# samiazirar/mvtracker

Hardware: AMD Instinct MI355X
Metric: query-points*frames/sec, 4-view 24-frame 512x512 @1024 queries (higher is better)
Workload: dtype bf16; 1 GPU; c3: 4-view synthetic 24-frame 512x512, 1024 queries, bf16 (configs[2], the metric's config); 4-view 24-frame 512x512, 1024 queries per GPU, corr K=16 x 4 levels, iters=4, 3 windows, random-init weights (seeded recipe); queries_total=1024, parallelism=query-shard x1, frame_store=bf16 rows

## Files before the change

### mvtracker_amd/csrc/block_fused.hip

```cpp
#include "common.h"
#include <stdlib.h>

namespace {

typedef __bf16 bf16x8 __attribute__((ext_vector_type(8)));
typedef __bf16 bf16x4 __attribute__((ext_vector_type(4)));
typedef unsigned u32x4 __attribute__((ext_vector_type(4)));
typedef unsigned u32x2 __attribute__((ext_vector_type(2)));

__device__ __forceinline__ void lds_barrier() {
#ifdef MVT_FULL_BARRIERS
  __syncthreads();
#else
  __builtin_amdgcn_fence(__ATOMIC_RELEASE, "workgroup", "local");
  __builtin_amdgcn_s_barrier();
  __builtin_amdgcn_fence(__ATOMIC_ACQUIRE, "workgroup", "local");
#endif
}

constexpr int NT = 512;
constexpr int C = 256;
constexpr int LDX = C + 8;
template <int NMB> struct Cfg {
  static constexpr int BM = 32 * NMB;
  static constexpr int HC = 256;
  static constexpr int JW = HC / 32;
  static constexpr int NM1 = NMB / (8 / JW);
  static constexpr int LDH = HC + 8;
  static constexpr int LDA = 296;
  static_assert(BM * LDA <= 2 * BM * LDH, "attention tile fits the H buffers");
};
constexpr int YLD = 40;
constexpr int NBIAS_DEAL = 4 * 256 + 256;
constexpr int FS = 512;

#ifdef MVT_STAMPS
__device__ unsigned long long mvt_stamp_buf[2 * 8 * 64];
#ifndef MVT_STAMP_SEL
#define MVT_STAMP_SEL true
#endif
#ifndef MVT_STAMP_WG1
#define MVT_STAMP_WG1 100
#endif
#define STAMP(i)                                                                                                  \
  do {                                                                                                            \
    __builtin_amdgcn_sched_barrier(0);                                                                            \
    unsigned long long t_;                                                                                        \
    asm volatile("s_memtime %0\n\ts_waitcnt lgkmcnt(0)" : "=s"(t_)::"memory");                                    \
    __builtin_amdgcn_sched_barrier(0);                                                                            \
    if (lane == 0 && MVT_STAMP_SEL && (bx == 0 || bx == MVT_STAMP_WG1) && by == 0 && bz == 0)  \
      mvt_stamp_buf[((bx ? 1 : 0) * 8 + wave) * 64 + (i)] = t_;                                                   \
  } while (0)
#else
#define STAMP(i) \
  do {           \
  } while (0)
#endif

#if defined(MVT_STAMPS) && defined(MVT_ASTAMPS)
#define ASTAMP(i)                                       \
  do {                                                  \
    const int wave = threadIdx.x >> 6;                  \
    const int bx = blockIdx.x, by = blockIdx.y, bz = blockIdx.z; \
    STAMP(i);                                           \
  } while (0)
#else
#define ASTAMP(i) \
  do {            \
  } while (0)
#endif

struct BlockArgs {
  float* x;
  int ldx;
  const float* att;
  int ldatt, Ko;
  const unsigned short* wo;
  const float* bo;
  int ldwo;
  const unsigned short* w1;
  const float* b1;
  const unsigned short* w2;
  const float* b2;
  int ldw1, ldw2, H;
  mvt_block_next next[MVT_BLOCK_MAX_NEXT];
  int n_next;
  int deal, deal_img[MVT_BLOCK_MAX_NEXT], deal_rep[2];
  int att_bf16;
  long long M;
  float* ws;
  const unsigned short* aq;
  const unsigned short* ak;
  const unsigned short* av;
  int ldaq, ldakv, S, nkeys, bmv;
  const float* parts;
  int nsplit;
  const float* tokx;
  const unsigned short* win;
  const float* bin;
  const float* virt;
  int ldtok;
  long long Mp;
  const float* t_coords;
  const float* t_fcorr;
  const float* t_ffeats;
  const float* t_maskvis;
  const float* t_pos;
  const float* t_time;
  int t_E, t_Fc, t_Cf, t_D;
  const float* c_ws;
  const float* c_b2;
  float* c_x;
  int c_ldx, c_nch;
  mvt_block_next c_kv;
  mvt_block_next c_next;
};

typedef float f32x2 __attribute__((ext_vector_type(2)));
__device__ __forceinline__ f32x2 gelu_tanh_pk(f32x2 x) {
  const f32x2 c0 = {-2.3022082f, -2.3022082f}, c1 = {-0.10294324f, -0.10294324f}, one = {1.0f, 1.0f};
  const f32x2 a = (x * x * c1 + c0) * x;
  f32x2 e;
  e[0] = __builtin_amdgcn_exp2f(a[0]);
  e[1] = __builtin_amdgcn_exp2f(a[1]);
  const f32x2 d = e + one;
  f32x2 rc;
  rc[0] = __builtin_amdgcn_rcpf(d[0]);
  rc[1] = __builtin_amdgcn_rcpf(d[1]);
  return x * rc;
}

__device__ __forceinline__ bf16x8 ldg_frag(const unsigned short* p) {
  return __builtin_bit_cast(bf16x8, *reinterpret_cast<const u32x4*>(p));
}
__device__ __forceinline__ bf16x8 lds_frag(const unsigned short* p) {
  return __builtin_bit_cast(bf16x8, *reinterpret_cast<const u32x4*>(p));
}

template <int KS, int NMB>
__device__ __forceinline__ void gemm_wt(f32x16 (&acc)[NMB], const unsigned short* wrow, const unsigned short* arow, int lda,
                                        int mb0) {
  constexpr int PF = (KS % 8 == 0) ? 8 : 4;
  bf16x8 wq[PF];
#pragma unroll
  for (int i = 0; i < PF; ++i) wq[i] = ldg_frag(wrow + (i < KS ? i : 0) * FS);
#pragma unroll 1
  for (int g = 0; g < KS / PF; ++g) {
#pragma unroll
    for (int j = 0; j < PF; ++j) {
      const int ks = g * PF + j;
      const bf16x8 wa = wq[j];
      wq[j] = ldg_frag(wrow + (ks + PF < KS ? ks + PF : KS - 1) * FS);
#pragma unroll
      for (int i = 0; i < NMB; ++i) {
        const bf16x8 xb = lds_frag(arow + (mb0 + i) * 32 * lda + ks * 16);
        acc[i] = __builtin_amdgcn_mfma_f32_32x32x16_bf16(wa, xb, acc[i], 0, 0, 0);
      }
    }
  }
#pragma unroll
  for (int j = 0; j < KS % PF; ++j) {
    const int ks = (KS / PF) * PF + j;
#pragma unroll
    for (int i = 0; i < NMB; ++i) {
      const bf16x8 xb = lds_frag(arow + (mb0 + i) * 32 * lda + ks * 16);
      acc[i] = __builtin_amdgcn_mfma_f32_32x32x16_bf16(wq[j], xb, acc[i], 0, 0, 0);
    }
  }
}

constexpr int PFQ = 16;
template <int KS, int NMB>
__device__ __forceinline__ void gemm_wq(f32x16 (&acc)[NMB], bf16x8 (&wq)[PFQ], const unsigned short* wrow, const unsigned short* nxt,
                                        const unsigned short* arow, int lda, int mb0) {
  static_assert(KS == PFQ, "every GEMM segment is exactly one queue length");
  constexpr int GK = NMB >= 2 ? 2 : 4;
  bf16x8 xa[GK][NMB], xn[GK][NMB];
// ... 5 lines not shown
  for (int g = 0; g < KS / GK; ++g) {
    if (g + 1 < KS / GK) {
#pragma unroll
      for (int j = 0; j < GK; ++j)
#pragma unroll
        for (int i = 0; i < NMB; ++i) xn[j][i] = lds_frag(arow + (mb0 + i) * 32 * lda + ((g + 1) * GK + j) * 16);
    }
    __builtin_amdgcn_sched_barrier(0);
#pragma unroll
    for (int j = 0; j < GK; ++j) {
      const int ks = g * GK + j;
      const bf16x8 wa = wq[ks];
#ifndef MVT_ABL_NOLOAD
      wq[ks] = ldg_frag(nxt + ks * FS);
#endif
#pragma unroll
      for (int i = 0; i < NMB; ++i) {
#ifdef MVT_ABL_NOLDS
        const bf16x8 xb = wa;
#else
        const bf16x8 xb = xa[j][i];
#endif
#ifdef MVT_ABL_NOMFMA
        acc[i][0] += (float)xb[0] + (float)wa[1];
#else
        acc[i] = __builtin_amdgcn_mfma_f32_32x32x16_bf16(wa, xb, acc[i], 0, 0, 0);
#endif
      }
    }
    __builtin_amdgcn_sched_barrier(0);
    if (g + 1 < KS / GK) {
#pragma unroll
      for (int j = 0; j < GK; ++j)
#pragma unroll
        for (int i = 0; i < NMB; ++i) xa[j][i] = xn[j][i];
    }
  }
}
template <int NMB, bool REFILL>
__device__ __forceinline__ void gemm_wq18(f32x16 (&acc)[NMB], bf16x8 (&wq)[PFQ], const bf16x8 (&wx)[2], const unsigned short* nxt,
                                          const unsigned short* arow, int lda) {
  constexpr int KS = 18, GK = 2;
  bf16x8 xa[GK][NMB], xn[GK][NMB];
#pragma unroll
  for (int j = 0; j < GK; ++j)
#pragma unroll
    for (int i = 0; i < NMB; ++i) xa[j][i] = lds_frag(arow + i * 32 * lda + j * 16);
#pragma unroll
  for (int g = 0; g < KS / GK; ++g) {
    if (g + 1 < KS / GK) {
#pragma unroll
      for (int j = 0; j < GK; ++j)
#pragma unroll
        for (int i = 0; i < NMB; ++i) xn[j][i] = lds_frag(arow + i * 32 * lda + ((g + 1) * GK + j) * 16);
    }
    __builtin_amdgcn_sched_barrier(0);
#pragma unroll
    for (int j = 0; j < GK; ++j) {
      const int ks = g * GK + j;
      const bf16x8 wa = ks < PFQ ? wq[ks < PFQ ? ks : 0] : wx[ks >= PFQ ? ks - PFQ : 0];
      if (REFILL && ks < PFQ) wq[ks] = ldg_frag(nxt + ks * FS);
#pragma unroll
      for (int i = 0; i < NMB; ++i) acc[i] = __builtin_amdgcn_mfma_f32_32x32x16_bf16(wa, xa[j][i], acc[i], 0, 0, 0);
    }
    __builtin_amdgcn_sched_barrier(0);
    if (g + 1 < KS / GK) {
#pragma unroll
      for (int j = 0; j < GK; ++j)
#pragma unroll
        for (int i = 0; i < NMB; ++i) xa[j][i] = xn[j][i];
    }
  }
}
__device__ __forceinline__ void fill_wq(bf16x8 (&wq)[PFQ], const unsigned short* wrow) {
#pragma unroll
  for (int j = 0; j < PFQ; ++j) wq[j] = ldg_frag(wrow + j * FS);
}

constexpr int LDVA = 40, DHA = 48, VTA = DHA * LDVA;
constexpr int LDKV = 584;
template <int NMBQ, int NKB> struct AttnFrags {
  u32x4 q[NMBQ][3];
  u32x4 k[NKB][3];
  u32x2 v[NKB][6];
};
template <int NMBQ, int NKB, class QR, class KR>
__device__ __forceinline__ void attn_load(AttnFrags<NMBQ, NKB>& f, const unsigned short* __restrict__ q, int ldq, QR qrow, int nq,
                                          const unsigned short* __restrict__ k, const unsigned short* __restrict__ v, int ldkv, KR krow,
                                          int nk, int hd, int lane) {
  const int r = lane & 31, h = lane >> 5;
#pragma unroll
  for (int mb = 0; mb < NMBQ; ++mb) {
    const int qi = mb * 32 + r;
    const long long qo = qrow(qi < nq ? qi : nq - 1) * (long long)ldq + hd * DHA;
#pragma unroll
    for (int ks = 0; ks < 3; ++ks) f.q[mb][ks] = *reinterpret_cast<const u32x4*>(q + qo + ks * 16 + 8 * h);
  }
#pragma unroll
  for (int kb = 0; kb < NKB; ++kb) {
    const int key = kb * 32 + r;
    const long long ko = krow(key < nk ? key : nk - 1) * (long long)ldkv + hd * DHA;
#pragma unroll
    for (int ks = 0; ks < 3; ++ks) f.k[kb][ks] = *reinterpret_cast<const u32x4*>(k + ko + ks * 16 + 8 * h);
#pragma unroll
    for (int i = 0; i < 6; ++i) f.v[kb][i] = *reinterpret_cast<const u32x2*>(v + ko + 24 * h + 4 * i);
  }
}
__device__ __forceinline__ f32x4 bf4_to_f32(unsigned lo, unsigned hi) {
  return (f32x4){__uint_as_float(lo << 16), __uint_as_float(lo & 0xFFFF0000u), __uint_as_float(hi << 16), __uint_as_float(hi & 0xFFFF0000u)};
}
__device__ __forceinline__ float pair_max(float v) {
  const auto r = __builtin_amdgcn_permlane32_swap(__float_as_int(v), __float_as_int(v), false, false);
  return fmaxf(__int_as_float(r[0]), __int_as_float(r[1]));
}
__device__ __forceinline__ float pair_sum(float v) {
  const auto r = __builtin_amdgcn_permlane32_swap(__float_as_int(v), __float_as_int(v), false, false);
  return __int_as_float(r[0]) + __int_as_float(r[1]);
}

template <int NMBQ, int NKB>
__device__ __forceinline__ void attn_compute(const AttnFrags<NMBQ, NKB>& f, int nq, int nk, int hd, unsigned short* vt,
                                             const unsigned short* zrow, unsigned short* As, int lda, int arow0, int lane, int bd = 0,
                                             int vstride = 0) {
  const int r = lane & 31, h = lane >> 5;
  const float scale = 1.0f / sqrtf((float)DHA);
  auto stage_vt = [&](int kb, unsigned short* img) {
    const int key = kb * 32 + r;
#pragma unroll
    for (int i = 0; i < 6; ++i) {
      u32x2 w = f.v[kb][i];
      if (key >= nk) w = (u32x2){0u, 0u};
#pragma unroll
      for (int e = 0; e < 4; ++e) img[(24 * h + 4 * i + e) * LDVA + r] = (unsigned short)((e & 1) ? (w[e >> 1] >> 16) : (w[e >> 1] & 0xFFFFu));
    }
  };
  if (vstride > 0) {
    __builtin_amdgcn_fence(__ATOMIC_SEQ_CST, "wavefront");
#pragma unroll
    for (int kb = 0; kb < NKB; ++kb) stage_vt(kb, vt + kb * vstride);
    __builtin_amdgcn_fence(__ATOMIC_SEQ_CST, "wavefront");
  }
  __builtin_amdgcn_sched_barrier(0);
  ASTAMP(49);
  bf16x8 qf[NMBQ][3];
#pragma unroll
  for (int mb = 0; mb < NMBQ; ++mb) {
#pragma unroll
    for (int ks = 0; ks < 3; ++ks) {
      f32x4 a = bf4_to_f32(f.q[mb][ks][0], f.q[mb][ks][1]), b = bf4_to_f32(f.q[mb][ks][2], f.q[mb][ks][3]);
#pragma unroll
      for (int e = 0; e < 4; ++e) {
        a[e] *= scale;
        b[e] *= scale;
      }
      const bf16x4 x = __builtin_convertvector(a, bf16x4), y = __builtin_convertvector(b, bf16x4);
#pragma unroll
      for (int e = 0; e < 4; ++e) {
        qf[mb][ks][e] = x[e];
        qf[mb][ks][4 + e] = y[e];
      }
    }
  }
  const unsigned bdm = bd > 0 ? (65536u / (unsigned)bd + 1u) : 0u;
#pragma unroll
  for (int mb = 0; mb < NMBQ; ++mb) {
    const int qi = mb * 32 + r;
    const unsigned qt = ((unsigned)qi * bdm) >> 16;
    f32x16 sc[NKB];
    float mx = -INFINITY;
#pragma unroll
    for (int kb = 0; kb < NKB; ++kb) {
#pragma unroll
      for (int e = 0; e < 16; ++e) sc[kb][e] = 0.f;
#pragma unroll
      for (int ks = 0; ks < 3; ++ks) sc[kb] = __builtin_amdgcn_mfma_f32_32x32x16_bf16(__builtin_bit_cast(bf16x8, f.k[kb][ks]), qf[mb][ks], sc[kb], 0, 0, 0);
    }
#pragma unroll
    for (int kb = 0; kb < NKB; ++kb) {
      const bool half = nk <= kb * 32 + 16;
#pragma unroll
      for (int e = 0; e < 16; ++e) {
        const unsigned kk = (unsigned)(kb * 32 + (e & 3) + 8 * (e >> 2)) + 4u * (unsigned)h;
        const bool ok = (kk < (unsigned)nk) & (((kk * bdm) >> 16) == qt);
        sc[kb][e] = ok ? sc[kb][e] : -INFINITY;
      }
#pragma unroll
      for (int e = 0; e < 8; ++e) mx = fmaxf(mx, sc[kb][e]);
      if (!half) {
#pragma unroll
        for (int e = 8; e < 16; ++e) mx = fmaxf(mx, sc[kb][e]);
      }
    }
    mx = pair_max(mx);
    if (mx == -INFINITY) mx = 0.f;
    float ps = 0.f;
#pragma unroll
    for (int kb = 0; kb < NKB; ++kb) {
      const bool half = nk <= kb * 32 + 16;
#pragma unroll
      for (int e = 0; e < 8; ++e) {
        sc[kb][e] = __expf(sc[kb][e] - mx);
        ps += sc[kb][e];
      }
      if (!half) {
#pragma unroll
        for (int e = 8; e < 16; ++e) {
          sc[kb][e] = __expf(sc[kb][e] - mx);
          ps += sc[kb][e];
        }
      }
    }
    __builtin_amdgcn_sched_barrier(0);
    ASTAMP(50 + 2 * mb);
    f32x16 oacc[2];
#pragma unroll
    for (int db = 0; db < 2; ++db)
#pragma unroll
      for (int e = 0; e < 16; ++e) oacc[db][e] = 0.f;
#pragma unroll
    for (int kb = 0; kb < NKB; ++kb) {
      const bool half = nk <= kb * 32 + 16;
      const unsigned short* vimg = vt + kb * vstride;
      if (vstride == 0 && (mb == 0 || NKB > 1)) {
        __builtin_amdgcn_fence(__ATOMIC_SEQ_CST, "wavefront");
        stage_vt(kb, vt);
        __builtin_amdgcn_fence(__ATOMIC_SEQ_CST, "wavefront");
      }
#pragma unroll
      for (int sk = 0; sk < 2; ++sk) {
        if (sk == 1 && half) break;
        f32x4 lo4, hi4;
#pragma unroll
        for (int e = 0; e < 4; ++e) {
          lo4[e] = sc[kb][8 * sk + e];
          hi4[e] = sc[kb][8 * sk + 4 + e];
        }
        const bf16x4 bl = __builtin_convertvector(lo4, bf16x4), bh = __builtin_convertvector(hi4, bf16x4);
        bf16x8 pb;
#pragma unroll
        for (int e = 0; e < 4; ++e) {
          pb[e] = bl[e];
          pb[4 + e] = bh[e];
        }
#pragma unroll
        for (int db = 0; db < 2; ++db) {
          const unsigned short* vr = (db * 32 + r < DHA) ? &vimg[(db * 32 + r) * LDVA + 16 * sk + 4 * h] : zrow + 16 * sk + 4 * h;
          const u32x2 a0 = *reinterpret_cast<const u32x2*>(vr), a1 = *reinterpret_cast<const u32x2*>(vr + 8);
          const bf16x8 va = __builtin_bit_cast(bf16x8, (u32x4){a0[0], a0[1], a1[0], a1[1]});
          oacc[db] = __builtin_amdgcn_mfma_f32_32x32x16_bf16(va, pb, oacc[db], 0, 0, 0);
        }
      }
    }
    __builtin_amdgcn_sched_barrier(0);
    ASTAMP(51 + 2 * mb);
    const float lt = pair_sum(ps);
    const float inv = 1.0f / lt;
    if (qi >= nq) continue;
#pragma unroll
    for (int db = 0; db < 2; ++db) {
#pragma unroll
      for (int gq = 0; gq < 4; ++gq) {
        const int d = db * 32 + 8 * gq + 4 * h;
        if (d < DHA) {
          f32x4 t;
#pragma unroll
          for (int e = 0; e < 4; ++e) t[e] = oacc[db][4 * gq + e] * inv;
          *reinterpret_cast<u32x2*>(&As[(arow0 + qi) * lda + hd * DHA + d]) = __builtin_bit_cast(u32x2, __builtin_convertvector(t, bf16x4));
        }
      }
    }
  }
}

template <int NMB>
__device__ __forceinline__ void ln_to_lds(const f32x16 (&v)[NMB], unsigned short* Xs, float* st, int wave, int lane, float eps,
                                          const float* lnw, const float* lnb, float (&ms)[NMB][2], bool have, bool sync = true) {
  constexpr int BM = 32 * NMB;
  const int r = lane & 31, h = lane >> 5;
  f32x4 gw[4], gb[4];
  if (lnw) {
#pragma unroll
    for (int g = 0; g < 4; ++g) {
      gw[g] = *reinterpret_cast<const f32x4*>(lnw + wave * 32 + 8 * g + 4 * h);
      gb[g] = *reinterpret_cast<const f32x4*>(lnb + wave * 32 + 8 * g + 4 * h);
    }
  }
  if (!have) {
#pragma unroll
    for (int mb = 0; mb < NMB; ++mb) {
      float s1 = 0.f, s2 = 0.f;
#pragma unroll
      for (int e = 0; e < 16; ++e) {
        s1 += v[mb][e];
        s2 = fmaf(v[mb][e], v[mb][e], s2);
      }
      s1 += __shfl_xor(s1, 32, 64);
      s2 += __shfl_xor(s2, 32, 64);
      if (h == 0) {
        st[(wave * BM + mb * 32 + r) * 2] = s1;
        st[(wave * BM + mb * 32 + r) * 2 + 1] = s2;
      }
    }
    lds_barrier();
#pragma unroll
    for (int mb = 0; mb < NMB; ++mb) {
      float s1 = 0.f, s2 = 0.f;
#pragma unroll
      for (int w = 0; w < 8; ++w) {
// ... 368 lines not shown
      const bool virt = m >= p.Mp;
      const long long tk = virt ? (m - p.Mp) / p.S : 0;
#pragma unroll
      for (int e = 0; e < 16; ++e) {
        const int c = wave * 32 + (e & 3) + 8 * (e >> 2) + 4 * h;
        v[mb][e] = virt ? p.virt[tk * C + c] : v[mb][e] + p.bin[c];
      }
    }
  } else if (MODE != 2 && ATT == 3) {
    unsigned short* As = &Hs[0][0];
    static_assert(ATT != 3 || NMB == 1, "partials tiles are 32 tokens");
    if (wave < 6) {
      const int mb = bx;
      const long long nchunk = (long long)p.S * 6;
      const long long cid = (long long)bz * 6 + wave;
      constexpr int MAXS = MVT_ATTN_NSPLIT;
      float ms[MAXS], ls[MAXS];
      f32x4 os[MAXS][2][4];
#pragma unroll
      for (int w = 0; w < MAXS; ++w) {
        const long long rec = (w < p.nsplit ? w : 0) * nchunk + cid;
        const f32x4 q0 = *reinterpret_cast<const f32x4*>(p.parts + mvt_part_off(rec, 0, lane));
        ms[w] = q0[mb];
        ls[w] = q0[2 + mb];
#pragma unroll
        for (int db = 0; db < 2; ++db)
#pragma unroll
          for (int g = 0; g < 4; ++g)
            os[w][db][g] = *reinterpret_cast<const f32x4*>(p.parts + mvt_part_off(rec, 1 + (mb * 2 + db) * 4 + g, lane));
      }
      __builtin_amdgcn_sched_barrier(0);
      float mm = ms[0], ll = ls[0];
      f32x16 oa[2];
#pragma unroll
      for (int db = 0; db < 2; ++db)
#pragma unroll
        for (int g = 0; g < 4; ++g)
#pragma unroll
          for (int e = 0; e < 4; ++e) oa[db][4 * g + e] = os[0][db][g][e];
#pragma unroll
      for (int w = 1; w < MAXS; ++w) {
        if (w >= p.nsplit) break;
        const float mw = ms[w];
        const float mn = fmaxf(mm, mw);
        const float ca = (mm == -INFINITY) ? 0.f : __expf(mm - mn);
        const float cb = (mw == -INFINITY) ? 0.f : __expf(mw - mn);
        ll = fmaf(ll, ca, ls[w] * cb);
#pragma unroll
        for (int db = 0; db < 2; ++db)
#pragma unroll
          for (int g = 0; g < 4; ++g)
#pragma unroll
            for (int e = 0; e < 4; ++e) oa[db][4 * g + e] = fmaf(oa[db][4 * g + e], ca, os[w][db][g][e] * cb);
        mm = mn;
      }
      const float inv = 1.0f / (ll + __shfl_xor(ll, 32, 64));
#pragma unroll
      for (int db = 0; db < 2; ++db)
#pragma unroll
        for (int g = 0; g < 4; ++g) {
          const int d = db * 32 + 8 * g + 4 * h;
          if (d < DHA) {
            f32x4 t4;
#pragma unroll
            for (int e = 0; e < 4; ++e) t4[e] = oa[db][4 * g + e] * inv;
            *reinterpret_cast<u32x2*>(&As[r * LDA + wave * DHA + d]) = __builtin_bit_cast(u32x2, __builtin_convertvector(t4, bf16x4));
          }
        }
    }
    pre_gemm();
    lds_barrier();
    gemm_wq18<NMB, HAS_MLP>(v, wq, wx, fc1_first, &As[r * LDA + 8 * h], LDA);
#pragma unroll
    for (int mb = 0; mb < NMB; ++mb)
#pragma unroll
      for (int e = 0; e < 16; ++e) v[mb][e] += p.bo[wave * 32 + (e & 3) + 8 * (e >> 2) + 4 * h];
  } else if (MODE != 2 && ATT != 0) {
    unsigned short* As = &Hs[0][0];
    unsigned short* zrow = reinterpret_cast<unsigned short*>(st);
    if (t < 48) zrow[t] = 0;
    constexpr int XW = (BM * LDX) / VTA;
    constexpr int VPW = NMB == 2 ? 2 : 1;
    constexpr int XWV = XW / VPW;
    unsigned short* vt = wave < XWV ? &Xs[wave * VPW * VTA] : &Hs[0][0] + ((BM * LDA + 7) & ~7) + (wave - XWV) * VPW * VTA;
    constexpr int vstride = VPW == 2 ? VTA : 0;
    static_assert(XWV + ((2 * BM * LDH - BM * LDA - 8) / VTA) / VPW >= 6, "the V^T images of six waves fit beside the attention tile");
    lds_barrier();
    STAMP(1);
    if (ATT == 1) {
      const long long left = p.M - m0;
      const int nrow = left < bmv ? (int)left : bmv;
      if (wave < 6 && nrow > 0) {
        auto row = [&](int j) { return m0 + j; };
        AttnFrags<NMB, 2> fr;
        attn_load<NMB, 2>(fr, p.aq, p.ldaq, row, nrow, p.ak, p.av, p.ldakv, row, nrow, wave, lane);
        attn_compute<NMB, 2>(fr, nrow, nrow, wave, vt, zrow, As, LDA, 0, lane, p.S, vstride);
      }
    } else {
      const bool on = wave < 6 && grow(0) >= 0;
      const long long left = ntok - (long long)bx * BM;
      const int nq = left < BM ? (int)left : BM;
      auto qrow = [&](int i) { return ((long long)bx * BM + i) * p.S + (long long)bz; };
      AttnFrags<NMB, 2> fr;
      if (CTX) {
        const unsigned short* KV = &Hs[0][0];
        auto krow = [&](int j) { return (long long)j; };
        if (on) attn_load<NMB, 2>(fr, p.aq, p.ldaq, qrow, nq, KV, KV + 288, LDKV, krow, p.nkeys, wave, lane);
        lds_barrier();
      } else {
        auto krow = [&](int j) { return (long long)j * p.S + (long long)bz; };
        if (on) attn_load<NMB, 2>(fr, p.aq, p.ldaq, qrow, nq, p.ak, p.av, p.ldakv, krow, p.nkeys, wave, lane);
      }
      if (on) attn_compute<NMB, 2>(fr, nq, p.nkeys, wave, vt, zrow, As, LDA, 0, lane, 0, vstride);
    }
    pre_gemm();
    STAMP(2);
    lds_barrier();
    STAMP(3);
    gemm_wq18<NMB, HAS_MLP>(v, wq, wx, fc1_first, &As[r * LDA + 8 * h], LDA);
#pragma unroll
    for (int mb = 0; mb < NMB; ++mb)
#pragma unroll
      for (int e = 0; e < 16; ++e) v[mb][e] += p.bo[wave * 32 + (e & 3) + 8 * (e >> 2) + 4 * h];
  } else if (MODE != 2 && p.att) {
    unsigned short* As = &Hs[0][0];
    const int q4 = p.Ko / 4;
    for (int f = t; f < BM * q4; f += NT) {
      const int row = f / q4, c = (f - row * q4) * 4;
      const long long m = grow(row);
      u32x2 w = (u32x2){0u, 0u};
      if (m >= 0) {
        if (p.att_bf16) {
          w = *reinterpret_cast<const u32x2*>(reinterpret_cast<const unsigned short*>(p.att) + m * (long long)p.ldatt + c);
        } else {
          const f32x4 a = *reinterpret_cast<const f32x4*>(p.att + m * (long long)p.ldatt + c);
          w = __builtin_bit_cast(u32x2, __builtin_convertvector(a, bf16x4));
        }
      }
      *reinterpret_cast<u32x2*>(&As[row * LDA + c]) = w;
    }
    pre_gemm();
    STAMP(2);
    lds_barrier();
    STAMP(3);
    gemm_wq18<NMB, HAS_MLP>(v, wq, wx, fc1_first, &As[r * LDA + 8 * h], LDA);
#pragma unroll
    for (int mb = 0; mb < NMB; ++mb)
#pragma unroll
      for (int e = 0; e < 16; ++e) v[mb][e] += p.bo[wave * 32 + (e & 3) + 8 * (e >> 2) + 4 * h];
  } else {
    load_x();
  }
  STAMP(4);
  if (MODE == 2 && p.ws) {
    constexpr int MAXCH = 4;
    const int nch = p.H / Cfg<NMB>::HC;
    f32x4 part[NMB][4][MAXCH + 1];
#pragma unroll
    for (int mb = 0; mb < NMB; ++mb) {
      const long long m = grow(mb * 32 + r);
#pragma unroll
      for (int g = 0; g < 4; ++g)
#pragma unroll
        for (int sidx = 0; sidx <= MAXCH; ++sidx)
          part[mb][g][sidx] = (m >= 0 && sidx <= nch) ? *reinterpret_cast<const f32x4*>(p.ws + ws_off(sidx, g)) : (f32x4){0.f, 0.f, 0.f, 0.f};
    }
    __builtin_amdgcn_sched_barrier(0);
#pragma unroll
    for (int mb = 0; mb < NMB; ++mb)
#pragma unroll
      for (int g = 0; g < 4; ++g) {
        f32x4 xv = part[mb][g][0];
#pragma unroll
        for (int sidx = 1; sidx <= MAXCH; ++sidx)
          if (sidx <= nch) {
#pragma unroll
            for (int e = 0; e < 4; ++e) xv[e] += part[mb][g][sidx][e];
          }
#pragma unroll
        for (int e = 0; e < 4; ++e) v[mb][4 * g + e] += xv[e] + p.b2[wave * 32 + 8 * g + 4 * h + e];
      }
  } else if (ATT != 4) {
#pragma unroll
    for (int mb = 0; mb < NMB; ++mb)
#pragma unroll
      for (int g = 0; g < 4; ++g)
#pragma unroll
        for (int e = 0; e < 4; ++e) v[mb][4 * g + e] += xr[mb][g][e];
  }

  auto store_x = [&]() {
#pragma unroll
    for (int mb = 0; mb < NMB; ++mb) {
      const long long m = grow(mb * 32 + r);
      if (m >= 0) {
#pragma unroll
        for (int g = 0; g < 4; ++g) {
          f32x4 o;
// ... 206 lines not shown
      for (int mb = 0; mb < NMB; ++mb)
#pragma unroll
        for (int e = 0; e < 16; ++e) acc[mb][e] = 0.f;
      gemm_wq<C / 16, NMB>(acc, wq, nrow_of(nb), nb + nbstep < nblocks ? nrow_of(nb + nbstep) : (chain ? chain : nrow_of(nb)), &Xs[r * LDX + 8 * h], LDX, 0);
      STAMP(34 + 8 * q + (nb - nb0) / nbstep);
      if (nx.y_bf16 && nb * 32 + 31 < nx.N && (nx.ldy & 7) == 0 && ((uintptr_t)nx.y & 15) == 0) {
        unsigned short* tile = &Hs[0][0] + wave * (NMB * 32 * YLD);
        __builtin_amdgcn_fence(__ATOMIC_SEQ_CST, "wavefront");
#pragma unroll
        for (int mb = 0; mb < NMB; ++mb)
#pragma unroll
          for (int g = 0; g < 4; ++g) {
            f32x4 o;
#pragma unroll
            for (int e = 0; e < 4; ++e) o[e] = acc[mb][4 * g + e] + b1s[nb * 32 + 8 * g + 4 * h + e];
            *reinterpret_cast<u32x2*>(&tile[(mb * 32 + r) * YLD + 8 * g + 4 * h]) = __builtin_bit_cast(u32x2, __builtin_convertvector(o, bf16x4));
          }
        __builtin_amdgcn_fence(__ATOMIC_SEQ_CST, "wavefront");
        unsigned short* yb = reinterpret_cast<unsigned short*>(nx.y) + nb * 32;
#pragma unroll
        for (int k = 0; k < NMB * 2; ++k) {
          const int pc = lane + 64 * k, row = pc >> 2, c = pc & 3;
          const long long m = grow(row);
          if (m >= nx.row_lo && m < nx.row_hi)
            *reinterpret_cast<u32x4*>(yb + m * (long long)nx.ldy + c * 8) = *reinterpret_cast<const u32x4*>(&tile[row * YLD + c * 8]);
        }
        continue;
      }
#pragma unroll
      for (int mb = 0; mb < NMB; ++mb) {
        const long long m = grow(mb * 32 + r);
        if (m < nx.row_lo || m >= nx.row_hi) continue;
#pragma unroll
        for (int g = 0; g < 4; ++g) {
          const int n = nb * 32 + 8 * g + 4 * h;
          if (n + 3 < nx.N) {
            f32x4 o;
#pragma unroll
            for (int e = 0; e < 4; ++e) o[e] = acc[mb][4 * g + e] + b1s[n + e];
            store_act4(nx.y, m * (long long)nx.ldy + n, o, nx.y_bf16);
          } else {
#pragma unroll
            for (int e = 0; e < 4; ++e)
              if (n + e < nx.N) store_act(nx.y, m * (long long)nx.ldy + n + e, acc[mb][4 * g + e] + b1s[n + e], nx.y_bf16);
          }
        }
      }
    }
    STAMP(39 + 8 * q);
  }
  STAMP(63);
}

__global__ void pack_frag_kernel(const unsigned short* __restrict__ w, int ld, int N, int K, unsigned short* __restrict__ out) {
  const long long total = (long long)((N + 31) / 32) * (K / 16) * 64;
  for (long long i = blockIdx.x * (long long)blockDim.x + threadIdx.x; i < total; i += (long long)gridDim.x * blockDim.x) {
    const int lane = (int)(i & 63);
    const long long f = i >> 6;
    const int ks = (int)(f % (K / 16));
    const int nb = (int)(f / (K / 16));
    const int n = nb * 32 + (lane & 31), k = ks * 16 + 8 * (lane >> 5);
    u32x4 v = (u32x4){0u, 0u, 0u, 0u};
    if (n < N) v = *reinterpret_cast<const u32x4*>(w + (long long)n * ld + k);
    *reinterpret_cast<u32x4*>(out + i * 8) = v;
  }
}

}

#ifdef MVT_STAMPS
extern "C" int mvt_debug_read_stamps(unsigned long long* host) {
  return hipMemcpyFromSymbol(host, HIP_SYMBOL(mvt_stamp_buf), sizeof(unsigned long long) * 2 * 8 * 64) == hipSuccess ? MVT_OK : MVT_ERR_HIP_BASE;
}
extern "C" int mvt_debug_clear_stamps() {
  static unsigned long long z[2 * 8 * 64];
  return hipMemcpyToSymbol(HIP_SYMBOL(mvt_stamp_buf), z, sizeof(z)) == hipSuccess ? MVT_OK : MVT_ERR_HIP_BASE;
}
#endif

static inline int proj_seq_switch() {
  const char* e = getenv("MVT_PROJ_SEQ");
  return e && atoi(e) != 0;
}
static void plan_deal(BlockArgs& a) {
  a.deal = 0;
  if (proj_seq_switch() || a.n_next == 0) return;
  int nimg = 0, total = 0;
  for (int q = 0; q < a.n_next; ++q) {
    const mvt_block_next& nx = a.next[q];
    if (!nx.y_bf16 || (nx.N & 31) || (nx.ldy & 7) || ((uintptr_t)nx.y & 15)) return;
    int im = -1;
    for (int qq = 0; qq < q && im < 0; ++qq)
      if (a.next[qq].lnw == nx.lnw && a.next[qq].lnb == nx.lnb && a.next[qq].eps == nx.eps) im = a.deal_img[qq];
    if (im < 0) {
      if (nimg == 2) return;
      im = nimg++;
      a.deal_rep[im] = q;
    }
    a.deal_img[q] = im;
    total += nx.N;
  }
  if (total <= NBIAS_DEAL) a.deal = 1;
}

extern "C" int mvt_pack_frag_bf16(const unsigned short* w, int ld, int N, int K, unsigned short* out, void* stream) {
  MVT_REQUIRE(w && out && N > 0 && K > 0 && K % 16 == 0 && ld % 8 == 0 && ld >= K);
  MVT_REQUIRE(((uintptr_t)w % 16 == 0) && ((uintptr_t)out % 16 == 0));
  const long long total = (long long)((N + 31) / 32) * (K / 16) * 64;
  hipLaunchKernelGGL(pack_frag_kernel, dim3((unsigned)mvt_cdiv(total, 256)), dim3(256), 0, mvt_stream(stream), w, ld, N, K, out);
  return mvt_launch_status();
}

extern "C" int mvt_block_fused_bf16(float* x, int ldx, const void* att, int att_bf16, int ldatt, int Ko, const unsigned short* wo, int ldwo,
                                    const float* bo, const unsigned short* w1, int ldw1, const float* b1, const unsigned short* w2,
                                    int ldw2, const float* b2, int H, const mvt_block_next* next, int n_next, long long M, int Cc,
                                    float* workspace, void* stream) {
  MVT_REQUIRE(x && w1 && b1 && w2 && b2 && M > 0 && Cc == C && H > 0 && H % 256 == 0 && H <= 4 * C);
  MVT_REQUIRE(ldx % 4 == 0 && ldx >= C);
  MVT_REQUIRE(!att || (wo && bo && Ko == 288 && ldatt % 4 == 0 && ldatt >= Ko));
  MVT_REQUIRE(n_next >= 0 && n_next <= MVT_BLOCK_MAX_NEXT && (n_next == 0 || next));
  MVT_REQUIRE(((uintptr_t)x % 16 == 0) && ((uintptr_t)att % 16 == 0) && ((uintptr_t)wo % 16 == 0) && ((uintptr_t)w1 % 16 == 0) &&
              ((uintptr_t)w2 % 16 == 0));
  BlockArgs a{};
  a.x = x; a.ldx = ldx; a.att = (const float*)att; a.att_bf16 = att_bf16 ? 1 : 0; a.ldatt = ldatt; a.Ko = Ko; a.wo = wo; a.bo = bo; a.ldwo = ldwo;
  a.w1 = w1; a.b1 = b1; a.w2 = w2; a.b2 = b2; a.ldw1 = ldw1; a.ldw2 = ldw2; a.H = H; a.M = M; a.n_next = n_next;
  for (int q = 0; q < n_next; ++q) {
    const mvt_block_next& nx = next[q];
    MVT_REQUIRE(nx.w && nx.b && nx.y && nx.N > 0 && nx.N <= 4 * C && nx.ldy % 4 == 0 && nx.ldy >= nx.N);
    MVT_REQUIRE(nx.y_bf16 == 0 || nx.y_bf16 == 1);
    MVT_REQUIRE((nx.lnw == nullptr) == (nx.lnb == nullptr) && ((uintptr_t)nx.lnw % 16 == 0) && ((uintptr_t)nx.lnb % 16 == 0) && ((uintptr_t)nx.w % 16 == 0) && ((uintptr_t)nx.y % 16 == 0));
    MVT_REQUIRE(nx.row_lo >= 0 && (nx.row_hi == 0 || nx.row_hi > nx.row_lo));
    a.next[q] = nx;
    if (nx.row_hi == 0) a.next[q].row_hi = M;
  }
  plan_deal(a);
  static const char* force = getenv("MVT_BLOCK_NMB");
  const int nmb = force ? atoi(force) : (M >= 4096 ? 2 : 1);
  static const bool no_split = getenv("MVT_BLOCK_NOSPLIT") != nullptr;
  a.ws = workspace;
  if (nmb == 2) {
    hipLaunchKernelGGL((block_fused_bf16<2, 0, 0>), dim3((unsigned)mvt_cdiv(M, 64)), dim3(NT), 0, mvt_stream(stream), a);
  } else if (workspace && !no_split && M <= 2048 && M % 32 == 0) {
    MVT_REQUIRE((uintptr_t)workspace % 16 == 0);
    const unsigned tiles = (unsigned)mvt_cdiv(M, 32);
    hipLaunchKernelGGL((block_fused_bf16<1, 1, 0>), dim3(tiles, (unsigned)(H / 256)), dim3(NT), 0, mvt_stream(stream), a);
    int maxblk = 1;
    for (int q = 0; q < n_next; ++q) maxblk = (next[q].N + 31) / 32 > maxblk ? (next[q].N + 31) / 32 : maxblk;
    const unsigned slices = n_next ? (unsigned)mvt_cdiv(maxblk, 8) : 1u;
    hipLaunchKernelGGL((block_fused_bf16<1, 2, 0>), dim3(tiles, slices), dim3(NT), 0, mvt_stream(stream), a);
  } else {
    hipLaunchKernelGGL((block_fused_bf16<1, 0, 0>), dim3((unsigned)mvt_cdiv(M, 32)), dim3(NT), 0, mvt_stream(stream), a);
  }
  return mvt_launch_status();
}

extern "C" int mvt_attn_block_fused_bf16(float* x, int ldx, const mvt_block_attn* attn, const unsigned short* wo, const float* bo,
                                         const unsigned short* w1, const float* b1, const unsigned short* w2, const float* b2, int H,
                                         const mvt_block_next* next, int n_next, long long M, int Cc, float* workspace, void* stream) {
  MVT_REQUIRE(x && attn && wo && bo && w1 && b1 && w2 && b2 && M > 0 && Cc == C && H > 0 && H % 256 == 0 && H <= 4 * C);
  MVT_REQUIRE(ldx % 4 == 0 && ldx >= C && n_next >= 0 && n_next <= MVT_BLOCK_MAX_NEXT && (n_next == 0 || next));
  MVT_REQUIRE(attn->heads == 6 && attn->dim_head == DHA && attn->S >= 1 && M % attn->S == 0);
  MVT_REQUIRE(attn->kind == MVT_ATTN_PARTIALS || (attn->kind == MVT_ATTN_FRAME_CTX && attn->q && attn->ldq % 8 == 0 && attn->ldq >= 288) ||
              (attn->q && attn->k && attn->v && attn->ldq % 8 == 0 && attn->ldkv % 8 == 0 && attn->ldq >= 288 && attn->ldkv >= 288));
  MVT_REQUIRE(((uintptr_t)x % 16 == 0) && ((uintptr_t)wo % 16 == 0) && ((uintptr_t)w1 % 16 == 0) && ((uintptr_t)w2 % 16 == 0));
  MVT_REQUIRE(((uintptr_t)attn->q % 16 == 0) && ((uintptr_t)attn->k % 16 == 0) && ((uintptr_t)attn->v % 16 == 0));
  BlockArgs a{};
  a.x = x; a.ldx = ldx; a.att = nullptr; a.Ko = 288; a.wo = wo; a.bo = bo; a.ldwo = 288;
  a.w1 = w1; a.b1 = b1; a.w2 = w2; a.b2 = b2; a.ldw1 = C; a.ldw2 = H; a.H = H; a.M = M; a.n_next = n_next; a.ws = workspace;
  a.aq = attn->q; a.ak = attn->k; a.av = attn->v; a.ldaq = attn->ldq; a.ldakv = attn->ldkv; a.S = attn->S; a.nkeys = attn->n_keys;
  for (int q = 0; q < n_next; ++q) {
    const mvt_block_next& nx = next[q];
    MVT_REQUIRE(nx.w && nx.b && nx.y && nx.N > 0 && nx.N <= 4 * C && nx.ldy % 4 == 0 && nx.ldy >= nx.N);
    MVT_REQUIRE((nx.y_bf16 == 0 || nx.y_bf16 == 1) && (nx.lnw == nullptr) == (nx.lnb == nullptr) && ((uintptr_t)nx.lnw % 16 == 0) && ((uintptr_t)nx.lnb % 16 == 0));
    MVT_REQUIRE(((uintptr_t)nx.w % 16 == 0) && ((uintptr_t)nx.y % 16 == 0) && nx.row_lo >= 0 && (nx.row_hi == 0 || nx.row_hi > nx.row_lo));
    a.next[q] = nx;
    if (nx.row_hi == 0) a.next[q].row_hi = M;
  }
  plan_deal(a);
  const int S = attn->S;
  if (attn->kind == MVT_ATTN_TIME) {
    MVT_REQUIRE(S <= 32 && !workspace);
    static const bool small_tiles = !(getenv("MVT_TIME_NMB1") && atoi(getenv("MVT_TIME_NMB1")) == 0);
    if (small_tiles && mvt_cdiv(M, (32 / S) * S) <= 256) {
      a.bmv = (32 / S) * S;
      hipLaunchKernelGGL((block_fused_bf16<1, 0, 1>), dim3((unsigned)mvt_cdiv(M, a.bmv)), dim3(NT), 0, mvt_stream(stream), a);
      return mvt_launch_status();
    }
    a.bmv = (64 / S) * S;
    hipLaunchKernelGGL((block_fused_bf16<2, 0, 1>), dim3((unsigned)mvt_cdiv(M, a.bmv)), dim3(NT), 0, mvt_stream(stream), a);
  } else if (attn->kind == MVT_ATTN_PARTIALS) {
    MVT_REQUIRE(attn->partials && attn->n_splits >= 1 && attn->n_splits <= MVT_ATTN_NSPLIT && attn->n_keys == 64 && M == 64LL * S);
    MVT_REQUIRE(workspace && (uintptr_t)workspace % 16 == 0 && M <= 2048 && (uintptr_t)attn->partials % 16 == 0);
    a.parts = attn->partials; a.nsplit = attn->n_splits;
    const unsigned tiles = (unsigned)mvt_cdiv(M, 32);
    a.S = S;
    hipLaunchKernelGGL((block_fused_bf16<1, 1, 3>), dim3(2, (unsigned)(H / 256), (unsigned)S), dim3(NT), 0, mvt_stream(stream), a);
    int maxblk = 1;
    for (int q = 0; q < n_next; ++q) maxblk = (next[q].N + 31) / 32 > maxblk ? (next[q].N + 31) / 32 : maxblk;
    const unsigned slices = n_next ? (unsigned)mvt_cdiv(maxblk, 8) : 1u;
    (void)tiles;
    if (!attn->defer_pass2)
      hipLaunchKernelGGL((block_fused_bf16<1, 2, 5>), dim3(2, slices, (unsigned)S), dim3(NT), 0, mvt_stream(stream), a);
  } else if (attn->kind == MVT_ATTN_FRAME) {
    MVT_REQUIRE(attn->n_keys >= 1 && attn->n_keys <= 64);
    const long long ntok = M / S;
    static const bool small_tiles = !(getenv("MVT_FRAME_NMB1") && atoi(getenv("MVT_FRAME_NMB1")) == 0);
    if (small_tiles && mvt_frame_small_tiles(ntok, S)) {
      MVT_REQUIRE(!workspace);
      hipLaunchKernelGGL((block_fused_bf16<1, 0, 2>), dim3((unsigned)mvt_cdiv(ntok, 32), 1, (unsigned)S), dim3(NT), 0, mvt_stream(stream), a);
    } else if (ntok * S >= 4096) {
      MVT_REQUIRE(!workspace);
      hipLaunchKernelGGL((block_fused_bf16<2, 0, 2>), dim3((unsigned)mvt_cdiv(ntok, 64), 1, (unsigned)S), dim3(NT), 0, mvt_stream(stream), a);
    } else {
      MVT_REQUIRE(workspace && (uintptr_t)workspace % 16 == 0 && M <= 2048 && ntok % 32 == 0);
      hipLaunchKernelGGL((block_fused_bf16<1, 1, 2>), dim3((unsigned)(ntok / 32), (unsigned)(H / 256), (unsigned)S), dim3(NT), 0,
                         mvt_stream(stream), a);
      int maxblk = 1;
      for (int q = 0; q < n_next; ++q) maxblk = (next[q].N + 31) / 32 > maxblk ? (next[q].N + 31) / 32 : maxblk;
      const unsigned slices = n_next ? (unsigned)mvt_cdiv(maxblk, 8) : 1u;
      if (!attn->defer_pass2)
        hipLaunchKernelGGL((block_fused_bf16<1, 2, 5>), dim3((unsigned)(ntok / 32), slices, (unsigned)S), dim3(NT), 0, mvt_stream(stream), a);
    }
  } else if (attn->kind == MVT_ATTN_FRAME_CTX) {
    const mvt_block_ctx* cx = attn->ctx;
    const long long ntok = M / S;
    MVT_REQUIRE(cx && attn->n_keys == 64 && ntok * S >= 4096 && !workspace && !attn->defer_pass2);
    MVT_REQUIRE(cx->ws && cx->b2 && cx->x && cx->chunks >= 1 && cx->chunks <= 4 && cx->ldx % 4 == 0 && cx->ldx >= C);
    MVT_REQUIRE(((uintptr_t)cx->ws % 16 == 0) && ((uintptr_t)cx->b2 % 16 == 0) && ((uintptr_t)cx->x % 16 == 0));
    MVT_REQUIRE(cx->kv.w && cx->kv.b && cx->kv.N == 2 * 288 && (cx->kv.lnw == nullptr) == (cx->kv.lnb == nullptr));
    MVT_REQUIRE(((uintptr_t)cx->kv.w % 16 == 0) && ((uintptr_t)cx->kv.lnw % 16 == 0) && ((uintptr_t)cx->kv.lnb % 16 == 0));
    const unsigned tiles = (unsigned)mvt_cdiv(ntok, 64);
    if (cx->next.w) {
      const mvt_block_next& nx = cx->next;
      MVT_REQUIRE(nx.b && nx.y && nx.N > 0 && nx.N <= 4 * C && nx.ldy % 4 == 0 && nx.ldy >= nx.N && (nx.y_bf16 == 0 || nx.y_bf16 == 1));
      MVT_REQUIRE((nx.lnw == nullptr) == (nx.lnb == nullptr) && ((uintptr_t)nx.lnw % 16 == 0) && ((uintptr_t)nx.lnb % 16 == 0));
      MVT_REQUIRE(((uintptr_t)nx.w % 16 == 0) && ((uintptr_t)nx.y % 16 == 0) && (nx.N + 31) / 32 <= 8 * (int)tiles);
    }
    a.c_ws = cx->ws; a.c_b2 = cx->b2; a.c_x = cx->x; a.c_ldx = cx->ldx; a.c_nch = cx->chunks; a.c_kv = cx->kv; a.c_next = cx->next;
    hipLaunchKernelGGL((block_fused_bf16<2, 0, 6>), dim3(tiles, 1, (unsigned)S), dim3(NT), 0, mvt_stream(stream), a);
  } else {
    return MVT_ERR_ARG;
  }
  return mvt_launch_status();
}

extern "C" int mvt_input_proj_bf16(const float* tokens, int ldtok, int token_dim, long long Mp, const unsigned short* win, const float* bin,
                                   const float* virtual_tokens, int S, float* x, int ldx, const mvt_block_next* next, int n_next, long long M,
                                   int Cc, void* stream) {
  MVT_REQUIRE(tokens && win && bin && virtual_tokens && x && next && n_next >= 1 && n_next <= MVT_BLOCK_MAX_NEXT && Cc == C);
  MVT_REQUIRE(M > 0 && Mp >= 0 && Mp <= M && S >= 1 && (M - Mp) % S == 0 && token_dim >= 1 && token_dim <= 37 * 16 && ldtok >= token_dim);
  MVT_REQUIRE(ldtok % 4 == 0 && ldx % 4 == 0 && ldx >= C && ((uintptr_t)tokens % 16 == 0) && ((uintptr_t)win % 16 == 0) && ((uintptr_t)x % 16 == 0));
  BlockArgs a{};
  a.x = x; a.ldx = ldx; a.M = M; a.n_next = n_next; a.H = 4 * C; a.ws = nullptr; a.S = S;
  a.tokx = tokens; a.ldtok = ldtok; a.win = win; a.bin = bin; a.virt = virtual_tokens; a.Mp = Mp;
  for (int q = 0; q < n_next; ++q) {
    const mvt_block_next& nx = next[q];
    MVT_REQUIRE(nx.w && nx.b && nx.y && nx.N > 0 && nx.N <= 4 * C && nx.ldy % 4 == 0 && nx.ldy >= nx.N);
    MVT_REQUIRE((nx.lnw == nullptr) == (nx.lnb == nullptr) && ((uintptr_t)nx.lnw % 16 == 0) && ((uintptr_t)nx.lnb % 16 == 0) && ((uintptr_t)nx.w % 16 == 0) && ((uintptr_t)nx.y % 16 == 0));
    MVT_REQUIRE(nx.row_lo >= 0 && (nx.row_hi == 0 || nx.row_hi > nx.row_lo) && (nx.y_bf16 == 0 || nx.y_bf16 == 1));
    a.next[q] = nx;
    if (nx.row_hi == 0) a.next[q].row_hi = M;
  }
  plan_deal(a);
  hipLaunchKernelGGL((block_fused_bf16<2, 3, 4>), dim3((unsigned)mvt_cdiv(M, 64)), dim3(NT), 0, mvt_stream(stream), a);
  return mvt_launch_status();
}

extern "C" int mvt_token_input_proj_bf16(const float* coords, const float* fcorr, int Fc, const float* ffeats, int Cf, const float* mask_vis,
                                         const float* pos, const float* time_embed, int n_tracks, int S, int E,
                                         const unsigned short* win, const float* bin, const float* virtual_tokens, float* x, int ldx,
                                         const mvt_block_next* next, int n_next, long long M, int Cc, void* stream) {
  MVT_REQUIRE(coords && fcorr && ffeats && mask_vis && pos && time_embed && win && bin && virtual_tokens && x && next);
  MVT_REQUIRE(n_next >= 1 && n_next <= MVT_BLOCK_MAX_NEXT && Cc == C && n_tracks > 0 && S >= 1 && E > 0 && E % 2 == 0 && Fc > 0 && Cf > 0);
  const int D = 3 * E + 3 + Fc + Cf + 2;
  const long long Mp = (long long)n_tracks * S;
  MVT_REQUIRE(D <= 37 * 16 && M >= Mp && (M - Mp) % S == 0 && ldx % 4 == 0 && ldx >= C);
  MVT_REQUIRE(((uintptr_t)win % 16 == 0) && ((uintptr_t)x % 16 == 0));
  BlockArgs a{};
  a.x = x; a.ldx = ldx; a.M = M; a.n_next = n_next; a.H = 4 * C; a.ws = nullptr; a.S = S;
  a.tokx = nullptr; a.win = win; a.bin = bin; a.virt = virtual_tokens; a.Mp = Mp;
  a.t_coords = coords; a.t_fcorr = fcorr; a.t_ffeats = ffeats; a.t_maskvis = mask_vis; a.t_pos = pos; a.t_time = time_embed;
  a.t_E = E; a.t_Fc = Fc; a.t_Cf = Cf; a.t_D = D;
  for (int q = 0; q < n_next; ++q) {
    const mvt_block_next& nx = next[q];
    MVT_REQUIRE(nx.w && nx.b && nx.y && nx.N > 0 && nx.N <= 4 * C && nx.ldy % 4 == 0 && nx.ldy >= nx.N);
    MVT_REQUIRE((nx.lnw == nullptr) == (nx.lnb == nullptr) && ((uintptr_t)nx.lnw % 16 == 0) && ((uintptr_t)nx.lnb % 16 == 0) && ((uintptr_t)nx.w % 16 == 0) && ((uintptr_t)nx.y % 16 == 0));
    MVT_REQUIRE(nx.row_lo >= 0 && (nx.row_hi == 0 || nx.row_hi > nx.row_lo) && (nx.y_bf16 == 0 || nx.y_bf16 == 1));
    a.next[q] = nx;
    if (nx.row_hi == 0) a.next[q].row_hi = M;
  }
  plan_deal(a);
  hipLaunchKernelGGL((block_fused_bf16<2, 3, 4>), dim3((unsigned)mvt_cdiv(M, 64)), dim3(NT), 0, mvt_stream(stream), a);
  return mvt_launch_status();
// ... 26 lines not shown
```

Before: 1.072 million query-points*frames/s.

## Split two attention heads across idle waves in 64-row fused block tiles

In the NMB=2 fused-block attention stage, only six of eight waves previously did head work. By default (attn_six off), waves 4-7 now split heads 4 and 5 by 32-query halves. Each cut wave stages its half of V^T and signals the partner through an LDS flag, and runs pre_gemm before its attention instead of after. V fragments are loaded as 16-byte vectors, and an env switch can force the 64-row tile path. This adds spin-wait flags and extra register and sync complexity to balance wave load.

```diff
diff --git a/mvtracker_amd/csrc/block_fused.hip b/mvtracker_amd/csrc/block_fused.hip
--- a/mvtracker_amd/csrc/block_fused.hip
+++ b/mvtracker_amd/csrc/block_fused.hip
@@ -62,7 +62,7 @@
   do {                                                  \
     const int wave = threadIdx.x >> 6;                  \
     const int bx = blockIdx.x, by = blockIdx.y, bz = blockIdx.z; \
-    STAMP(i);                                           \
+    STAMP((i) + 7);                                     \
   } while (0)
 #else
 #define ASTAMP(i) \
@@ -93,6 +93,7 @@
   const unsigned short* ak;
   const unsigned short* av;
   int ldaq, ldakv, S, nkeys, bmv;
+  int attn_six;
   const float* parts;
   int nsplit;
   const float* tokx;
@@ -264,16 +265,16 @@
 template <int NMBQ, int NKB> struct AttnFrags {
   u32x4 q[NMBQ][3];
   u32x4 k[NKB][3];
-  u32x2 v[NKB][6];
+  u32x4 v[NKB][3];
 };
 template <int NMBQ, int NKB, class QR, class KR>
 __device__ __forceinline__ void attn_load(AttnFrags<NMBQ, NKB>& f, const unsigned short* __restrict__ q, int ldq, QR qrow, int nq,
                                           const unsigned short* __restrict__ k, const unsigned short* __restrict__ v, int ldkv, KR krow,
-                                          int nk, int hd, int lane) {
+                                          int nk, int hd, int lane, int q0 = 0, int vkb = -1) {
   const int r = lane & 31, h = lane >> 5;
 #pragma unroll
   for (int mb = 0; mb < NMBQ; ++mb) {
-    const int qi = mb * 32 + r;
+    const int qi = q0 + mb * 32 + r;
     const long long qo = qrow(qi < nq ? qi : nq - 1) * (long long)ldq + hd * DHA;
 #pragma unroll
     for (int ks = 0; ks < 3; ++ks) f.q[mb][ks] = *reinterpret_cast<const u32x4*>(q + qo + ks * 16 + 8 * h);
@@ -284,8 +285,27 @@
     const long long ko = krow(key < nk ? key : nk - 1) * (long long)ldkv + hd * DHA;
 #pragma unroll
     for (int ks = 0; ks < 3; ++ks) f.k[kb][ks] = *reinterpret_cast<const u32x4*>(k + ko + ks * 16 + 8 * h);
-#pragma unroll
-    for (int i = 0; i < 6; ++i) f.v[kb][i] = *reinterpret_cast<const u32x2*>(v + ko + 24 * h + 4 * i);
+    if (vkb < 0) {
+#pragma unroll
+      for (int i = 0; i < 3; ++i) f.v[kb][i] = *reinterpret_cast<const u32x4*>(v + ko + 24 * h + 8 * i);
+    }
+  }
+  if (vkb >= 0) {
+    const int key = vkb * 32 + r;
+    const long long vo = krow(key < nk ? key : nk - 1) * (long long)ldkv + hd * DHA;
+#pragma unroll
+    for (int i = 0; i < 3; ++i) f.v[0][i] = *reinterpret_cast<const u32x4*>(v + vo + 24 * h + 8 * i);
+  }
+}
+__device__ __forceinline__ void attn_stage_vt(const u32x4 (&v)[3], int kb, int nk, unsigned short* img, int lane) {
+  const int r = lane & 31, h = lane >> 5;
+  const int key = kb * 32 + r;
+#pragma unroll
+  for (int i = 0; i < 6; ++i) {
+    u32x2 w = (u32x2){v[i >> 1][2 * (i & 1)], v[i >> 1][2 * (i & 1) + 1]};
+    if (key >= nk) w = (u32x2){0u, 0u};
+#pragma unroll
+    for (int e = 0; e < 4; ++e) img[(24 * h + 4 * i + e) * LDVA + r] = (unsigned short)((e & 1) ? (w[e >> 1] >> 16) : (w[e >> 1] & 0xFFFFu));
   }
 }
 __device__ __forceinline__ f32x4 bf4_to_f32(unsigned lo, unsigned hi) {
@@ -300,28 +320,22 @@
   return __int_as_float(r[0]) + __int_as_float(r[1]);
 }
 
+__device__ __forceinline__ void lds_flag_set(int* flag) {
+  __builtin_amdgcn_fence(__ATOMIC_RELEASE, "workgroup", "local");
+  __hip_atomic_store(flag, 1, __ATOMIC_RELAXED, __HIP_MEMORY_SCOPE_WORKGROUP);
+}
+__device__ __forceinline__ void lds_flag_wait(int* flag) {
+#pragma clang loop unroll(disable)
+  for (int i = 0; i < (1 << 20) && __hip_atomic_load(flag, __ATOMIC_RELAXED, __HIP_MEMORY_SCOPE_WORKGROUP) == 0; ++i) __builtin_amdgcn_s_sleep(1);
+  __builtin_amdgcn_fence(__ATOMIC_ACQUIRE, "workgroup", "local");
+}
+
 template <int NMBQ, int NKB>
 __device__ __forceinline__ void attn_compute(const AttnFrags<NMBQ, NKB>& f, int nq, int nk, int hd, unsigned short* vt,
                                              const unsigned short* zrow, unsigned short* As, int lda, int arow0, int lane, int bd = 0,
-                                             int vstride = 0) {
+                                             int vstride = 0, int q0 = 0, int* vready = nullptr) {
   const int r = lane & 31, h = lane >> 5;
   const float scale = 1.0f / sqrtf((float)DHA);
-  auto stage_vt = [&](int kb, unsigned short* img) {
-    const int key = kb * 32 + r;
-#pragma unroll
-    for (int i = 0; i < 6; ++i) {
-      u32x2 w = f.v[kb][i];
-      if (key >= nk) w = (u32x2){0u, 0u};
-#pragma unroll
-      for (int e = 0; e < 4; ++e) img[(24 * h + 4 * i + e) * LDVA + r] = (unsigned short)((e & 1) ? (w[e >> 1] >> 16) : (w[e >> 1] & 0xFFFFu));
-    }
-  };
-  if (vstride > 0) {
-    __builtin_amdgcn_fence(__ATOMIC_SEQ_CST, "wavefront");
-#pragma unroll
-    for (int kb = 0; kb < NKB; ++kb) stage_vt(kb, vt + kb * vstride);
-    __builtin_amdgcn_fence(__ATOMIC_SEQ_CST, "wavefront");
-  }
   __builtin_amdgcn_sched_barrier(0);
   ASTAMP(49);
   bf16x8 qf[NMBQ][3];
@@ -346,7 +360,7 @@
   const unsigned bdm = bd > 0 ? (65536u / (unsigned)bd + 1u) : 0u;
 #pragma unroll
   for (int mb = 0; mb < NMBQ; ++mb) {
-    const int qi = mb * 32 + r;
+    const int qi = q0 + mb * 32 + r;
     const unsigned qt = ((unsigned)qi * bdm) >> 16;
     f32x16 sc[NKB];
     float mx = -INFINITY;
@@ -394,6 +408,7 @@
     }
     __builtin_amdgcn_sched_barrier(0);
     ASTAMP(50 + 2 * mb);
+    if (vready) lds_flag_wait(vready);
     f32x16 oacc[2];
 #pragma unroll
     for (int db = 0; db < 2; ++db)
@@ -405,7 +420,7 @@
       const unsigned short* vimg = vt + kb * vstride;
       if (vstride == 0 && (mb == 0 || NKB > 1)) {
         __builtin_amdgcn_fence(__ATOMIC_SEQ_CST, "wavefront");
-        stage_vt(kb, vt);
+        attn_stage_vt(f.v[kb], kb, nk, vt, lane);
         __builtin_amdgcn_fence(__ATOMIC_SEQ_CST, "wavefront");
       }
 #pragma unroll
@@ -940,38 +955,70 @@
     constexpr int XW = (BM * LDX) / VTA;
     constexpr int VPW = NMB == 2 ? 2 : 1;
     constexpr int XWV = XW / VPW;
-    unsigned short* vt = wave < XWV ? &Xs[wave * VPW * VTA] : &Hs[0][0] + ((BM * LDA + 7) & ~7) + (wave - XWV) * VPW * VTA;
     constexpr int vstride = VPW == 2 ? VTA : 0;
-    static_assert(XWV + ((2 * BM * LDH - BM * LDA - 8) / VTA) / VPW >= 6, "the V^T images of six waves fit beside the attention tile");
+    static_assert(XWV + ((2 * BM * LDH - BM * LDA - 8) / VTA) / VPW >= 6, "the V^T images of six heads fit beside the attention tile");
+    const bool six = NMB != 2 || p.attn_six != 0;
+    const bool whole = wave < (six ? 6 : 4), cut = !six && wave >= 4;
+    const int hd = whole ? wave : 4 + (wave & 1);
+    const int cq = (wave - 4) >> 1;
+    int* vflag = reinterpret_cast<int*>(st) + 32;
+    if (NMB == 2 && t < 4) vflag[t] = 0;
+    unsigned short* vt = hd < XWV ? &Xs[hd * VPW * VTA] : &Hs[0][0] + ((BM * LDA + 7) & ~7) + (hd - XWV) * VPW * VTA;
     lds_barrier();
     STAMP(1);
+    auto attention = [&](auto qrow, int nq, const unsigned short* kp, const unsigned short* vp, int ldkv, auto krow, int nk, int bd, bool any,
+                         bool operands_in_lds) {
+      AttnFrags<NMB, 2> fr;
+      AttnFrags<1, 2> fc;
+      if (any && whole) attn_load<NMB, 2>(fr, p.aq, p.ldaq, qrow, nq, kp, vp, ldkv, krow, nk, hd, lane);
+      if constexpr (NMB == 2) {
+        if (any && cut) attn_load<1, 2>(fc, p.aq, p.ldaq, qrow, nq, kp, vp, ldkv, krow, nk, hd, lane, 32 * cq, cq);
+      }
+      if (operands_in_lds) lds_barrier();
+      if constexpr (NMB == 2) {
+        __builtin_amdgcn_fence(__ATOMIC_SEQ_CST, "wavefront");
+        if (any && whole) {
+#pragma unroll
+          for (int kb = 0; kb < 2; ++kb) attn_stage_vt(fr.v[kb], kb, nk, vt + kb * vstride, lane);
+        }
+        if (any && cut) {
+          attn_stage_vt(fc.v[0], cq, nk, vt + cq * vstride, lane);
+          lds_flag_set(&vflag[2 * (hd - 4) + cq]);
+        }
+        __builtin_amdgcn_fence(__ATOMIC_SEQ_CST, "wavefront");
+        ASTAMP(54);
+        if (!cut) {
+          if (any && whole) attn_compute<NMB, 2>(fr, nq, nk, hd, vt, zrow, As, LDA, 0, lane, bd, vstride);
+          pre_gemm();
+        } else {
+          pre_gemm();
+          __builtin_amdgcn_sched_barrier(0);
+          if (any && 32 * cq < nq)
+            attn_compute<1, 2>(fc, nq, nk, hd, vt, zrow, As, LDA, 0, lane, bd, vstride, 32 * cq, &vflag[2 * (hd - 4) + (cq ^ 1)]);
+        }
+      } else {
+        if (any && whole) attn_compute<NMB, 2>(fr, nq, nk, hd, vt, zrow, As, LDA, 0, lane, bd, 0);
+      }
+    };
     if (ATT == 1) {
       const long long left = p.M - m0;
       const int nrow = left < bmv ? (int)left : bmv;
-      if (wave < 6 && nrow > 0) {
-        auto row = [&](int j) { return m0 + j; };
-        AttnFrags<NMB, 2> fr;
-        attn_load<NMB, 2>(fr, p.aq, p.ldaq, row, nrow, p.ak, p.av, p.ldakv, row, nrow, wave, lane);
-        attn_compute<NMB, 2>(fr, nrow, nrow, wave, vt, zrow, As, LDA, 0, lane, p.S, vstride);
-      }
+      auto row = [&](int j) { return m0 + j; };
+      attention(row, nrow, p.ak, p.av, p.ldakv, row, nrow, p.S, nrow > 0, false);
     } else {
-      const bool on = wave < 6 && grow(0) >= 0;
       const long long left = ntok - (long long)bx * BM;
       const int nq = left < BM ? (int)left : BM;
       auto qrow = [&](int i) { return ((long long)bx * BM + i) * p.S + (long long)bz; };
-      AttnFrags<NMB, 2> fr;
       if (CTX) {
         const unsigned short* KV = &Hs[0][0];
         auto krow = [&](int j) { return (long long)j; };
-        if (on) attn_load<NMB, 2>(fr, p.aq, p.ldaq, qrow, nq, KV, KV + 288, LDKV, krow, p.nkeys, wave, lane);
-        lds_barrier();
+        attention(qrow, nq, KV, KV + 288, LDKV, krow, p.nkeys, 0, grow(0) >= 0, true);
       } else {
         auto krow = [&](int j) { return (long long)j * p.S + (long long)bz; };
-        if (on) attn_load<NMB, 2>(fr, p.aq, p.ldaq, qrow, nq, p.ak, p.av, p.ldakv, krow, p.nkeys, wave, lane);
-      }
-      if (on) attn_compute<NMB, 2>(fr, nq, p.nkeys, wave, vt, zrow, As, LDA, 0, lane, 0, vstride);
-    }
-    pre_gemm();
+        attention(qrow, nq, p.ak, p.av, p.ldakv, krow, p.nkeys, 0, grow(0) >= 0, false);
+      }
+    }
+    if (NMB != 2) pre_gemm();
     STAMP(2);
     lds_barrier();
     STAMP(3);
@@ -1344,6 +1391,14 @@
   const char* e = getenv("MVT_PROJ_SEQ");
   return e && atoi(e) != 0;
 }
+static inline int attn_six_switch() {
+  const char* e = getenv("MVT_ATTN_SIX");
+  return e && atoi(e) != 0;
+}
+static inline int attn_tile64_switch() {
+  const char* e = getenv("MVT_ATTN_TILE64");
+  return e && atoi(e) != 0;
+}
 static void plan_deal(BlockArgs& a) {
   a.deal = 0;
   if (proj_seq_switch() || a.n_next == 0) return;
@@ -1430,6 +1485,8 @@
   a.x = x; a.ldx = ldx; a.att = nullptr; a.Ko = 288; a.wo = wo; a.bo = bo; a.ldwo = 288;
   a.w1 = w1; a.b1 = b1; a.w2 = w2; a.b2 = b2; a.ldw1 = C; a.ldw2 = H; a.H = H; a.M = M; a.n_next = n_next; a.ws = workspace;
   a.aq = attn->q; a.ak = attn->k; a.av = attn->v; a.ldaq = attn->ldq; a.ldakv = attn->ldkv; a.S = attn->S; a.nkeys = attn->n_keys;
+  a.attn_six = attn_six_switch();
+  const bool tile64 = attn_tile64_switch() != 0;
   for (int q = 0; q < n_next; ++q) {
     const mvt_block_next& nx = next[q];
     MVT_REQUIRE(nx.w && nx.b && nx.y && nx.N > 0 && nx.N <= 4 * C && nx.ldy % 4 == 0 && nx.ldy >= nx.N);
@@ -1443,7 +1500,7 @@
   if (attn->kind == MVT_ATTN_TIME) {
     MVT_REQUIRE(S <= 32 && !workspace);
     static const bool small_tiles = !(getenv("MVT_TIME_NMB1") && atoi(getenv("MVT_TIME_NMB1")) == 0);
-    if (small_tiles && mvt_cdiv(M, (32 / S) * S) <= 256) {
+    if (small_tiles && !tile64 && mvt_cdiv(M, (32 / S) * S) <= 256) {
       a.bmv = (32 / S) * S;
       hipLaunchKernelGGL((block_fused_bf16<1, 0, 1>), dim3((unsigned)mvt_cdiv(M, a.bmv)), dim3(NT), 0, mvt_stream(stream), a);
       return mvt_launch_status();
@@ -1467,10 +1524,10 @@
     MVT_REQUIRE(attn->n_keys >= 1 && attn->n_keys <= 64);
     const long long ntok = M / S;
     static const bool small_tiles = !(getenv("MVT_FRAME_NMB1") && atoi(getenv("MVT_FRAME_NMB1")) == 0);
-    if (small_tiles && mvt_frame_small_tiles(ntok, S)) {
+    if (small_tiles && !tile64 && mvt_frame_small_tiles(ntok, S)) {
       MVT_REQUIRE(!workspace);
       hipLaunchKernelGGL((block_fused_bf16<1, 0, 2>), dim3((unsigned)mvt_cdiv(ntok, 32), 1, (unsigned)S), dim3(NT), 0, mvt_stream(stream), a);
-    } else if (ntok * S >= 4096) {
+    } else if (ntok * S >= 4096 || (tile64 && !workspace)) {
       MVT_REQUIRE(!workspace);
       hipLaunchKernelGGL((block_fused_bf16<2, 0, 2>), dim3((unsigned)mvt_cdiv(ntok, 64), 1, (unsigned)S), dim3(NT), 0, mvt_stream(stream), a);
     } else {
```

After: 1.067 million query-points*frames/s. No clear change (-0.5%).
